# spotify/basic-pitch

Hardware: NVIDIA H100
Metric: audio_seconds_per_second (higher is better)
Workload: dtype f32

## Files before the change

basic_pitch_b200/csrc/kernels.cuh:

```cuda
#pragma once
#include <cuda_bf16.h>

#include <cstring>
#include <vector>

#include "common.cuh"

namespace bp {

void hcqt_setup();
constexpr int kLp2 = kTaps + 14;
struct Lowpass2 {
  float2 t[kLp2];
};
Lowpass2 lowpass_pairs(const float* h_lp );
void launch_decimate(const Lowpass2& lp, const float* audio, const WinDesc* desc, float* chain, int stage, int n_windows,
                     cudaStream_t st);
void launch_cqt(const float* audio, const WinDesc* desc, const float* chain, const float* wt, const float* scale,
                float* logmag, unsigned int* minmax, int n_windows, cudaStream_t st);
void launch_lognorm(float* y, const unsigned int* minmax, const float* bn , int n_windows,
                    cudaStream_t st);

struct CnnWeights {
  const float *contour1_wT, *contour1_b;
  const float *contour2_wT, *contour2_b;
  const float *note1_wT, *note1_b;
  const float *note2_wT, *note2_b;
  const float *onset1_wT, *onset1_b;
  const float *onset2_wT, *onset2_b;
};
void cnn_setup();
void launch_contour1(const float* y, const CnnWeights& w, float* c1, int n_windows, cudaStream_t st);
void launch_contour2(const float* c1, const CnnWeights& w, float* contour, int n_windows, cudaStream_t st);
void launch_note1(const float* contour, const CnnWeights& w, float* n1, int n_windows, cudaStream_t st);
void launch_note2(const float* n1, const CnnWeights& w, float* note, int n_windows, cudaStream_t st);
void launch_onset1(const float* y, const CnnWeights& w, float* o1, int n_windows, cudaStream_t st);
void launch_onset2(const float* note, const float* o1, const CnnWeights& w, float* onset, int n_windows,
                   cudaStream_t st);


struct TcConvSpec {
  int KH, KW, SF, PT, PL, COUT, FLT, WOUT;
  int n_ci;
  int shifts[8];
  int data_bins, chunks8;
  int rows_per_window, lead_rows;
  int layer;
  int KH2, HALO, G0;
  int n2_tiles, n2, js, width, pass;
  int W;
  int slot[24];
  __host__ __device__ constexpr int n_ft() const { return (WOUT + FLT - 1) / FLT; }
  __host__ __device__ constexpr int tile_bins() const { return 8 * (chunks8 - 1); }
  __host__ __device__ constexpr int ksteps() const { return (KH * n_ci * W + 15) / 16; }
  __host__ __device__ constexpr int edge_per_side() const { return 2 * HALO + (layer == 0 ? 8 - HALO : 0); }
};
__host__ __device__ constexpr TcConvSpec tc_spec(int layer) {
  return layer == 0 ? TcConvSpec{3, 39, 1, 1, 19, 8, 16, 264, 8, {-36, 0, 36, 57, 72, 84, 93, 101}, kCqtBins,     40, 174, 3, 0, 5, 2, 9,  1, 32, 5, 104, 40, 0, {}}
       : layer == 1 ? TcConvSpec{5, 5, 3, 2, 1, 32, 4, 88, 8, {-36, 0, 36, 57, 72, 84, 93, 101},   kCqtBins,     40, 174, 3, 1, 3, 1, 12, 2, 16, 4, 32, 32,   6,
                                 {9, 10, 21, 22, 14, 4, 2, 1, 16, 3, 6, 13, 5, 17, 18, 20, 19, 23, 7, 0, 8, 15, 12, 11}}
                    : TcConvSpec{7, 7, 3, 3, 2, 32, 4, 88, 1, {0, 0, 0, 0, 0, 0, 0, 0},           kContourBins, 34, 175, 6, 2, 7, 1, 12, 2, 32, 8, 64, 64,   8, {}};
}
struct TcConvPlan {
  TcConvSpec spec{};
  std::vector<uint16_t> tiles;
  std::vector<int> tile_seq;
  std::vector<uint32_t> slot_words[2];
  std::vector<int> group_step_off;
  std::vector<int> group_ft;
  int n_tiles = 0, n_groups = 0, n_uses = 0;
  void build(const TcConvSpec& spec, const float* w );
};
struct TcConvDev {
  int layer;
  const uint16_t* tiles;
  const uint16_t* b1;
  const uint16_t* b2;
  float bias1[32];
  float bias2;
  float note_w[9];
};
int tc_upload_program(const TcConvPlan& contour_plan, cudaStream_t st);
void tc_build_b1(int layer, const float* w, std::vector<uint16_t>& out, bool window8 = false);
struct TcGatherGeom {
  int K, n_ci, KH, wout;
  int K_packed;
  std::vector<int> starts, ranges;
  std::vector<int> kmap;
};
TcGatherGeom tc_gather_geometry(int layer);
void tc_build_b2(int layer, const float* w2, std::vector<uint16_t>& out);
void tc_build_b2_full(int layer, const float* w2, std::vector<uint16_t>& out);
int tc_rows_total(int n_windows, int rows_per_window);
size_t tc_edge_floats(const TcConvSpec& spec, int n_windows);
// ... 172 lines not shown
```

basic_pitch_b200/csrc/tc_conv.cu:

```cuda
#include <cuda.h>
#include <cuda_bf16.h>

#include <algorithm>
#include <cstdlib>
#include <cstring>
#include <unordered_map>
#include <vector>

#include "kernels.cuh"
#include "tc_ptx.cuh"

namespace bp {

namespace tc {
constexpr int kMTile = 64;
constexpr int kTileBytes = 8192;
constexpr int kMaxSteps = 1024;
constexpr int kMaxGroups = 15;
static_assert(tc_spec(0).G0 <= kMaxGroups, "contour groups in constant memory");
constexpr int kConsumerWarps = 8;
constexpr int kProducerWarp = 8;
constexpr int kThreads = 32 * kConsumerWarps + 128;
constexpr int kProducerRegs = 24;
constexpr int kConsumerRegs = 240;
static_assert(kProducerRegs + 2 * kConsumerRegs <= 3 * 168, "register pool of the CTA");
}

__host__ __device__ constexpr int tc_gather_k(TcConvSpec g, int dt, int ci, int j) {
  if (g.W == 8) return 8 * (dt * g.n_ci + ci) + j;
  int P = 0;
  while (g.slot[P] != 3 * ci + j / 2) ++P;
  return g.n_ci * g.W * dt + 2 * P + (j & 1);
}
__host__ __device__ constexpr bool tc_gather_slots_ok(TcConvSpec g) {
  if (g.W == 8) return true;
  if (g.W != 6 || g.n_ci != 8) return false;
  for (int p = 0; p < 24; ++p) {
    int n = 0;
    for (int P = 0; P < 24; ++P) n += g.slot[P] == p;
    if (n != 1) return false;
  }
  return true;
}
__host__ __device__ constexpr int tc_gather_slot_shift(TcConvSpec g, int P) { return g.shifts[g.slot[P] / 3]; }
__host__ __device__ constexpr int tc_gather_slot_pair(TcConvSpec g, int P) { return g.slot[P] % 3; }
static_assert(tc_gather_slots_ok(tc_spec(1)) && tc_gather_slots_ok(tc_spec(2)), "K slot map of the gather");
static_assert(tc_spec(1).ksteps() == 15 && tc_spec(2).ksteps() == 4, "K-steps per output bin");
__host__ __device__ constexpr int tc_gather_start(TcConvSpec g, int f, int ci) {
  return (g.SF * f - g.PL + g.shifts[ci]) & ~1;
}
__host__ __device__ constexpr int tc_gather_lo(TcConvSpec g, int ci) { return g.shifts[ci] > 0 ? g.shifts[ci] : 0; }
__host__ __device__ constexpr int tc_gather_hi(TcConvSpec g, int ci) {
// ... 26 lines not shown
  return s;
}
static_assert(tc_smem(0, false).stages == 12 && tc_smem(0, true).stages == 9, "weight-ring depth per layer");
static_assert(tc_smem(1, true).total() <= kMaxSmem && tc_smem(2, true).total() <= kMaxSmem, "onset / note shared memory");
constexpr uint32_t kUseFirstAcc = 1u << 15, kNoUse = 0xffffffffu;
}

static inline uint16_t f2bf(float x) {
  uint32_t u;
  memcpy(&u, &x, 4);
  if ((u & 0x7f800000u) == 0x7f800000u) return (uint16_t)(u >> 16);
  u += 0x7fffu + ((u >> 16) & 1u);
  return (uint16_t)(u >> 16);
}
static inline float bf2f(uint16_t h) {
  uint32_t u = (uint32_t)h << 16;
  float f;
  memcpy(&f, &u, 4);
  return f;
}

void TcConvPlan::build(const TcConvSpec& sp, const float* W ) {
  using namespace tc;
  spec = sp;
  tiles.clear();
  tile_seq.clear();
  slot_words[0].clear();
  slot_words[1].clear();
  group_step_off.clear();
  group_ft.clear();
  const int n_ft = sp.n_ft();
  const int data_rows = kMTile + sp.KH - 1;
  const int lbo16 = data_rows;
  const int stride = sp.G0;

  std::unordered_map<uint64_t, std::vector<int>> by_hash;
  int n_keys = 0;
  std::vector<uint16_t> scratch(kTileBytes / 2);
  std::vector<uint32_t> key(16 * 128), keys;
  auto find_or_add = [&](int dt, int c, int ft, int clip_lo) -> int {
    bool any = false;
    std::fill(scratch.begin(), scratch.end(), (uint16_t)0);
    std::fill(key.begin(), key.end(), 0u);
    for (int kk = clip_lo; kk < 16; ++kk) {
      const int u = 8 * c + kk;
      if (u >= sp.data_bins) continue;
      for (int n = 0; n < 128; ++n) {
        const int fl = n / sp.COUT, co = n % sp.COUT;
        const int f = ft * sp.FLT + fl;
        double acc = 0.0;
        uint32_t mask = 0;
        for (int ci = 0; ci < sp.n_ci; ++ci) {
          const int gg = u - sp.shifts[ci];
          const int df = gg - sp.SF * f + sp.PL;
          if (df < 0 || df >= sp.KW || gg < 0 || gg >= kContourBins) continue;
          acc += (double)W[((co * sp.n_ci + ci) * sp.KH + dt) * sp.KW + df];
          mask |= 1u << ci;
        }
        if (!mask) continue;
        key[kk * 128 + n] = 1u + (((uint32_t)(dt * 1024 + (u - sp.SF * f + 512)) << 8) | mask);
        const float w = (float)acc;
        const uint16_t hi = f2bf(w);
        const uint16_t lo = f2bf(w - bf2f(hi));
        const size_t o = (size_t)(kk >> 3) * 128 * 8 + (size_t)n * 8 + (kk & 7);
        scratch[o] = hi;
        scratch[2048 + o] = lo;
        any = true;
      }
    }
    if (!any) return -1;
    uint64_t h = 1469598103934665603ull;
    for (uint32_t v : key) h = (h ^ v) * 1099511628211ull;
    for (int id : by_hash[h])
      if (std::memcmp(keys.data() + (size_t)id * key.size(), key.data(), key.size() * 4) == 0) return id;
    tiles.insert(tiles.end(), scratch.begin(), scratch.end());
    keys.insert(keys.end(), key.begin(), key.end());
    by_hash[h].push_back(n_keys);
    return n_keys++;
  };

  group_step_off.push_back(0);
  n_uses = 0;
  for (int ft_a = 0; ft_a < stride; ++ft_a) {
    const int ft_b = ft_a + stride < n_ft ? ft_a + stride : -1;
    const int fts[2] = {ft_a, ft_b};
    group_ft.push_back(ft_a);
    group_ft.push_back(ft_b);
    struct Use {
      int tile, slot, c8, dt, off;
    };
    std::vector<Use> uses;
    for (int dt = 0; dt < sp.KH; ++dt) {
      std::vector<Use> cand;
      for (int slot = 0; slot < 2; ++slot) {
        const int ft = fts[slot];
        if (ft < 0) continue;
        std::vector<bool> need(sp.chunks8, false);
        for (int ci = 0; ci < sp.n_ci; ++ci)
          for (int fl = 0; fl < sp.FLT; ++fl) {
            const int f = ft * sp.FLT + fl;
            if (f >= sp.WOUT) continue;
            for (int df = 0; df < sp.KW; ++df) {
              const int gg = sp.SF * f - sp.PL + df, u = gg + sp.shifts[ci];
              if (gg < 0 || gg >= kContourBins || u < 0 || u >= sp.data_bins) continue;
              need[u / 8] = true;
            }
          }
        for (int c8 = 0; c8 < sp.chunks8;) {
          if (!need[c8]) {
            ++c8;
            continue;
          }
          const int c = std::min(c8, sp.chunks8 - 3);
          const int off = 8 * c - sp.SF * sp.FLT * ft;
          const int tile = find_or_add(dt, c, ft, 8 * (c8 - c));
          if (tile >= 0) cand.push_back(Use{tile, slot, c, dt, off});
          c8 += 2;
        }
      }
      std::stable_sort(cand.begin(), cand.end(), [](const Use& a, const Use& b) {
        return a.off != b.off ? a.off < b.off : (a.tile != b.tile ? a.tile < b.tile : a.slot < b.slot);
      });
      uses.insert(uses.end(), cand.begin(), cand.end());
    }
    struct Step {
      int tile;
      uint32_t w[2];
    };
    std::vector<Step> steps;
    size_t i = 0;
    while (i < uses.size()) {
      size_t j = i;
      while (j < uses.size() && uses[j].tile == uses[i].tile && (j == i || uses[j].slot != uses[j - 1].slot)) ++j;
      Step stp{uses[i].tile, {kNoUse, kNoUse}};
      for (size_t u = i; u < j; ++u) {
        stp.w[uses[u].slot] = (uint32_t)(uses[u].c8 * lbo16 + uses[u].dt);
        ++n_uses;
      }
      steps.push_back(stp);
      i = j;
    }
    std::stable_sort(steps.begin(), steps.end(), [](const Step& a, const Step& b) {
      auto cls = [](const Step& s) { return s.w[1] == kNoUse ? 0 : (s.w[0] == kNoUse ? 2 : 1); };
      return cls(a) < cls(b);
    });
    bool seen[2] = {false, false};
    for (Step& stp : steps) {
      for (int sl = 0; sl < 2; ++sl)
        if (stp.w[sl] != kNoUse) {
          if (!seen[sl]) stp.w[sl] |= kUseFirstAcc;
          seen[sl] = true;
        }
      tile_seq.push_back(stp.tile);
      slot_words[0].push_back(stp.w[0]);
      slot_words[1].push_back(stp.w[1]);
    }
    group_step_off.push_back((int)tile_seq.size());
  }
  n_tiles = n_keys;
  n_groups = (int)group_ft.size() / 2;
}

__constant__ uint32_t c_prog[2][tc::kMaxSteps];
__constant__ int c_tile_seq[tc::kMaxSteps];
__constant__ int c_group_step_off[tc::kMaxGroups + 1];
__constant__ int c_group_ft[2 * tc::kMaxGroups];

void tc_build_b2(int layer, const float* w2, std::vector<uint16_t>& out) {
  const TcConvSpec sp = tc_spec(layer);
  const int tile_elems = 2 * 16 * sp.n2, KW2 = 2 * sp.HALO + 1;
  out.assign((size_t)sp.n2_tiles * tile_elems, 0);
  for (int tl = 0; tl < sp.n2_tiles; ++tl)
    for (int kk = 0; kk < 16; ++kk)
      for (int n = 0; n < sp.n2; ++n) {
        const int jp = n / sp.js, dt = n - jp * sp.js;
        const int b = (16 * tl + kk) / sp.COUT, c = (16 * tl + kk) % sp.COUT, df = b + 2 * sp.HALO - jp;
        if (dt >= sp.KH2 || df < 0 || df >= KW2) continue;
        const float w = w2[((c + (layer == 1 ? 1 : 0)) * sp.KH2 + dt) * KW2 + df];
        const uint16_t hi = f2bf(w), lo = f2bf(w - bf2f(hi));
        const size_t o = (size_t)tl * tile_elems + (size_t)(kk >> 3) * sp.n2 * 8 + (size_t)n * 8 + (kk & 7);
        out[o] = hi;
        out[o + 16 * sp.n2] = lo;
      }
}

int tc_upload_program(const TcConvPlan& pl, cudaStream_t st) {
  if (pl.spec.layer != 0 || (int)pl.tile_seq.size() > tc::kMaxSteps - 1 || pl.n_groups != tc_spec(0).G0) return -1;
  for (int sl = 0; sl < 2; ++sl)
    cudaMemcpyToSymbolAsync(c_prog, pl.slot_words[sl].data(), pl.slot_words[sl].size() * 4, (size_t)sl * tc::kMaxSteps * 4,
                            cudaMemcpyHostToDevice, st);
  cudaMemcpyToSymbolAsync(c_tile_seq, pl.tile_seq.data(), pl.tile_seq.size() * 4, 0, cudaMemcpyHostToDevice, st);
  cudaMemcpyToSymbolAsync(c_group_step_off, pl.group_step_off.data(), pl.group_step_off.size() * 4, 0,
                          cudaMemcpyHostToDevice, st);
  cudaMemcpyToSymbolAsync(c_group_ft, pl.group_ft.data(), pl.group_ft.size() * 4, 0, cudaMemcpyHostToDevice, st);
  return cudaStreamSynchronize(st) == cudaSuccess ? 0 : -1;
}

void tc_build_b1(int layer, const float* W , std::vector<uint16_t>& out, bool window8) {
  const TcConvSpec g = tc_spec(layer);
  const int wn = window8 ? 8 : g.W;
  const size_t plane = (size_t)16 * ((g.KH * g.n_ci * wn + 15) / 16) * 32;
  out.assign(4 * plane, 0);
  for (int p = 0; p < 2; ++p)
    for (int dt = 0; dt < g.KH; ++dt)
      for (int ci = 0; ci < g.n_ci; ++ci) {
        const int o = g.SF * p - g.PL + g.shifts[ci] - tc_gather_start(g, p, ci);
        for (int j = 0; j < wn; ++j) {
          const int df = j - o, k = window8 ? 8 * (dt * g.n_ci + ci) + j : tc_gather_k(g, dt, ci, j);
          if (df < 0 || df >= g.KW) continue;
          for (int co = 0; co < 32; ++co) {
            const float w = W[((co * g.n_ci + ci) * g.KH + dt) * g.KW + df];
            const uint16_t hi = f2bf(w), lo = f2bf(w - bf2f(hi));
            const size_t e = ((size_t)(k >> 3) * 32 + co) * 8 + (k & 7);
            out[(2 * p) * plane + e] = hi;
            out[(2 * p + 1) * plane + e] = lo;
          }
        }
      }
}

TcGatherGeom tc_gather_geometry(int layer) {
  const TcConvSpec g = tc_spec(layer);
  TcGatherGeom r;
  r.K = 16 * ((g.KH * g.n_ci * 8 + 15) / 16);
  r.K_packed = 16 * g.ksteps();
  for (int k = 0; k < r.K_packed; ++k) {
    int hit[3] = {-1, -1, -1};
// ... 146 lines not shown
};
#endif

int tc_read_clocks(int layer, unsigned long long* out, bool reset) {
#ifdef BP_TC_CLOCKS
  if (layer < 0 || layer > 2) return -1;
  if (cudaMemcpyFromSymbol(out, g_tc_clocks, tc::kNumClk * sizeof(unsigned long long),
                           (size_t)layer * tc::kNumClk * sizeof(unsigned long long)) != cudaSuccess)
    return -1;
  if (reset) {
    static const unsigned long long zero[tc::kNumClk] = {};
    if (cudaMemcpyToSymbol(g_tc_clocks, zero, sizeof(zero), (size_t)layer * sizeof(zero)) != cudaSuccess) return -1;
  }
  return 0;
#else
  (void)layer, (void)out, (void)reset;
  return -1;
#endif
}

__device__ __forceinline__ void slot_barrier(int slot) {
  asm volatile("bar.sync %0, 128;" ::"r"(1 + slot) : "memory");
}


struct RowOut {
  float* raw;
  float* unw;
  __nv_bfloat16* chl;
  float* edge;
  const float* note_col;
  int t;
  bool ok;
  int e_lo, e_hi;
};

template <int LAYER>
__device__ __forceinline__ void finish_pitch_tile(const TcArgs& a, const RowOut& ro, float (&S)[6], float (&carry)[2], int ft,
                                                  bool first, bool last) {
  constexpr TcConvSpec L = tc_spec(LAYER);
  static_assert(L.FLT + 2 * L.HALO == 6 && L.HALO == 1, "sums and carry of a pitch tile");
  const bool lower = ft > 0;
  if (first) {
    if (lower && ro.edge) {
      float* e = ro.edge + (size_t)(ro.e_lo * 2 + 0) * L.edge_per_side() * a.edge_rows;
      e[0] = S[0];
      e[a.edge_rows] = S[1];
    }
  } else {
    S[0] += carry[0];
    S[1] += carry[1];
  }
  const int jlo = first ? (lower ? 2 * L.HALO : L.HALO) : 0;
  const int jhi = (ft == L.n_ft() - 1) ? L.FLT + L.HALO : L.FLT;
  if (ro.ok) {
    float nv[3][6];
    if constexpr (LAYER == 1) {
#pragma unroll
      for (int c = 0; c < 6; ++c) {
        const int f = L.FLT * ft - 2 + c;
        const bool fin = (unsigned)f < (unsigned)kPitches;
        const float* col = ro.note_col + (size_t)f * a.o.raw_rows;
#pragma unroll
        for (int r = 0; r < 3; ++r)
          nv[r][c] = (fin && (unsigned)(ro.t + r - 1) < (unsigned)kFrames) ? __ldg(col + r - 1) : 0.f;
      }
    }
#pragma unroll
    for (int j = 0; j < L.FLT + L.HALO; ++j) {
      if (j < jlo || j >= jhi) continue;
      const int f = L.FLT * ft - L.HALO + j;
      float x = S[j] + a.bias2;
      if constexpr (LAYER == 1) {
#pragma unroll
        for (int r = 0; r < 3; ++r)
#pragma unroll
          for (int df = 0; df < 3; ++df)
            if (j + df < 6) x = fmaf(nv[r][j + df], a.note_w[r * 3 + df], x);
      }
      const float v = sigmoidf_fast(x);
      if (ro.raw) ro.raw[(size_t)f * a.o.raw_rows] = v;
      if (ro.unw) ro.unw[(size_t)f * a.o.frame_stride] = v;
    }
  }
  carry[0] = S[L.FLT];
  carry[1] = S[L.FLT + 1];
  if (last && ft < L.n_ft() - 1 && ro.edge && ro.e_hi >= 0) {
    float* e = ro.edge + (size_t)(ro.e_hi * 2 + 1) * L.edge_per_side() * a.edge_rows;
    e[0] = S[L.FLT];
    e[a.edge_rows] = S[L.FLT + 1];
  }
}

__device__ __forceinline__ void store_contour_chunk(const TcArgs& a, const RowOut& ro, int chunk, const float (&v)[8]) {
  store_split8(v, ro.chl, (size_t)chunk * a.o.chl_rows * 8, (size_t)a.o.chl_chunks * a.o.chl_rows * 8);
  const float4 x0 = make_float4(v[0], v[1], v[2], v[3]), x1 = make_float4(v[4], v[5], v[6], v[7]);
  if (ro.raw) {
    float4* d = reinterpret_cast<float4*>(ro.raw + (size_t)chunk * a.o.raw_rows * 8);
    d[0] = x0;
    d[1] = x1;
  }
  if (ro.unw) {
    float4* d = reinterpret_cast<float4*>(ro.unw + (size_t)chunk * a.o.frame_stride * 8);
    d[0] = x0;
    d[1] = x1;
  }
}

__device__ __forceinline__ void finish_contour_tile(const TcArgs& a, const RowOut& ro, float (&S)[20], int ft, bool first,
                                                    bool last, float (&carry)[4], float (&hold)[6]) {
  constexpr TcConvSpec L = tc_spec(0);
  static_assert(L.FLT == 16 && L.HALO == 2 && L.edge_per_side() == 10, "sums, carry and edge values of a contour tile");
  const bool lower = ft > 0;
  if (first) {
    if (lower && ro.edge) {
      float* e = ro.edge + (size_t)(ro.e_lo * 2 + 0) * L.edge_per_side() * a.edge_rows;
#pragma unroll
      for (int k = 0; k < 4; ++k) e[(size_t)k * a.edge_rows] = S[k];
#pragma unroll
      for (int k = 0; k < 6; ++k) e[(size_t)(4 + k) * a.edge_rows] = sigmoidf_fast(S[4 + k] + a.bias2);
    }
  } else {
#pragma unroll
    for (int k = 0; k < 4; ++k) S[k] += carry[k];
  }
  float fin[16];
#pragma unroll
  for (int j = 0; j < 16; ++j) fin[j] = sigmoidf_fast(S[j] + a.bias2);
  if (ro.ok) {
    if (!first) {
      const float v[8] = {hold[0], hold[1], hold[2], hold[3], hold[4], hold[5], fin[0], fin[1]};
      store_contour_chunk(a, ro, 2 * ft - 1, v);
    }
    if (!first || !lower) {
      const float v[8] = {fin[2], fin[3], fin[4], fin[5], fin[6], fin[7], fin[8], fin[9]};
      store_contour_chunk(a, ro, 2 * ft, v);
    }
  }
#pragma unroll
  for (int k = 0; k < 6; ++k) hold[k] = fin[10 + k];
#pragma unroll
  for (int k = 0; k < 4; ++k) carry[k] = S[16 + k];
  if (last && ft < L.n_ft() - 1 && ro.edge && ro.e_hi >= 0) {
    float* e = ro.edge + (size_t)(ro.e_hi * 2 + 1) * L.edge_per_side() * a.edge_rows;
#pragma unroll
    for (int k = 0; k < 4; ++k) e[(size_t)k * a.edge_rows] = S[16 + k];
#pragma unroll
    for (int k = 0; k < 6; ++k) e[(size_t)(4 + k) * a.edge_rows] = fin[10 + k];
  }
}

template <int NW>
__device__ __forceinline__ void conv2_mma(float (&p)[NW / 2], const uint32_t (&ah)[32], const uint32_t (&al)[32], uint32_t b2) {
  constexpr uint32_t kPlane = 128u * NW * 2u;
#pragma unroll
  for (int ks = 0; ks < 8; ++ks) {
    const uint64_t bh = make_desc(b2 + (uint32_t)(2 * ks * NW * 16), NW * 16, 128);
    const uint64_t bl = make_desc(b2 + kPlane + (uint32_t)(2 * ks * NW * 16), NW * 16, 128);
    const uint32_t xh[4] = {ah[4 * ks], ah[4 * ks + 1], ah[4 * ks + 2], ah[4 * ks + 3]};
    const uint32_t xl[4] = {al[4 * ks], al[4 * ks + 1], al[4 * ks + 2], al[4 * ks + 3]};
    if constexpr (NW == 104) {
      wgmma_rs_n104(p, xh, bh, ks ? 1u : 0u);
      wgmma_rs_n104(p, xh, bl, 1u);
      wgmma_rs_n104(p, xl, bh, 1u);
    } else if constexpr (NW == 64) {
      wgmma_rs_n64(p, xh, bh, ks ? 1u : 0u);
      wgmma_rs_n64(p, xh, bl, 1u);
      wgmma_rs_n64(p, xl, bh, 1u);
    } else {
      wgmma_rs_n32(p, xh, bh, ks ? 1u : 0u);
      wgmma_rs_n32(p, xh, bl, 1u);
      wgmma_rs_n32(p, xl, bh, 1u);
    }
  }
}

template <int LAYER>
// ... 82 lines not shown
    gr.template load<(I + 2) % KS>(s_data, x[(I + 2) % 3]);
    clk.lap(kClkFull);
  }
  if constexpr (I + 1 < NST) gather_steps<LAYER, I + 1>(acc, gr, x, s_data, d0, ft, fr0, qd, clk);
}

template <int LAYER>
__device__ __forceinline__ void gather_conv1(float (&acc)[64], const unsigned char* s_data, uint32_t b1, int ft, int fr0, int qd,
                                             TcClocks& clk) {
  using namespace tc;
  static_assert(tc_spec(LAYER).ksteps() >= 2, "the first two K-steps are loaded up front, of the same bin");
  GatherRegs<LAYER> gr;
  const uint64_t d0 = make_desc(b1, 32 * 16, 128);
  uint32_t x[3][8];
  gr.setup(tc_spec(LAYER).FLT * ft, fr0, qd);
  gr.template load<0>(s_data, x[0]);
  gr.template load<1>(s_data, x[1]);
  clk.lap(kClkFull);
  gather_steps<LAYER, 0>(acc, gr, x, s_data, d0, ft, fr0, qd, clk);
  wgmma_wait<0>();
  reg_fence(acc);
  clk.lap(kClkMma);
}

template <int LAYER, bool FUSED>
__global__ void __launch_bounds__(tc::kThreads, 1) conv_tc_kernel(const __grid_constant__ TcArgs a) {
  using namespace tc;
  constexpr TcConvSpec L = tc_spec(LAYER);
  constexpr bool kFused = FUSED;
  constexpr bool kGather = LAYER != 0;
  static_assert(kFused || !kGather, "the onset and note epilogues always fuse the next conv");
  constexpr int NW = L.width, PC = L.pass, PS = PC + 1;
  static_assert(PC % 8 == 0 && PC % L.js == 0, "a staging pass holds whole fragment blocks and whole output offsets");
  constexpr int kDataRows = kMTile + L.KH - 1, kFt = L.n_ft();
  extern __shared__ __align__(128) unsigned char smem[];
  constexpr TcSmem SM = tc_smem(LAYER, FUSED);
  constexpr int kStages = SM.stages;
  static_assert(SM.total() <= kMaxSmem && kStages <= kMaxStages && (kGather || kStages >= 4), "dynamic shared memory per CTA");
  unsigned char* s_data = smem;
  unsigned char* s_w = smem + SM.data_bytes;
  unsigned char* s_b1 = s_w + kStages * kTileBytes;
  unsigned char* s_b2 = s_b1 + SM.b1_bytes;
  float* s_p = reinterpret_cast<float*>(s_b2 + SM.b2_bytes);
  uint64_t* bars = reinterpret_cast<uint64_t*>(reinterpret_cast<unsigned char*>(s_p) + SM.p_bytes);
  uint64_t* full_w = bars;
  uint64_t* empty_w = bars + kStages;
  uint64_t* data_full = bars + 2 * kStages;
  uint64_t* data_empty = data_full + 1;
  uint64_t* b2_full = data_empty + 1;
  uint64_t* b1_full = b2_full + 1;
  uint32_t* issued = reinterpret_cast<uint32_t*>(b1_full + 1);

  const int warp = __shfl_sync(0xffffffffu, (int)(threadIdx.x >> 5), 0);
  const int lane = threadIdx.x & 31;
  constexpr uint32_t lbo = kDataRows * 16u;
  constexpr uint32_t plane_bytes = (L.chunks8 - 1) * lbo;

  if (threadIdx.x == 0) {
    for (int s = 0; s < kStages; ++s) {
      mbar_init(full_w + s, 1);
      mbar_init(empty_w + s, kConsumerWarps);
    }
    mbar_init(data_full, 1);
    mbar_init(data_empty, kConsumerWarps);
    mbar_init(b2_full, 1);
    mbar_init(b1_full, 1);
    *issued = 0;
// ... 54 lines not shown
    }
    clk.lap(kClkProdOther);
    clk.flush(LAYER);
  } else {
    setmaxnreg_inc<kConsumerRegs>();
    const int slot = warp >> 2, wq = warp & 3, gq = lane >> 2, qd = lane & 3;
    const int tid = threadIdx.x & 127;
    const int fr0 = 16 * wq + gq;
    uint32_t stage = 0, ph_w = 0, ph_d = 0, n_fill = 0;
    const uint32_t a_hi = smem_u32(s_data), a_lo = a_hi + plane_bytes, w_base = smem_u32(s_w);
    const uint32_t* prog = c_prog[slot];
    float* sp_rows = s_p + slot * 64 * PS;
    if constexpr (kFused) mbar_wait_wd(b2_full, 0, 6);
    if constexpr (kGather) mbar_wait_wd(b1_full, 0, 7);
    for (int it = blockIdx.x; it < n_items; it += gridDim.x) {
      const int mt = it / a.n_split, spl = it % a.n_split;
      const int g0 = spl * L.G0 / a.n_split, g1 = (spl + 1) * L.G0 / a.n_split;
      bool live[2];
      int rb[2], rt[2];
#pragma unroll
      for (int rr = 0; rr < 2; ++rr) {
        const int m = mt * a.ms - a.h2 + fr0 + 8 * rr;
        rb[rr] = m >= 0 ? m / L.rows_per_window : 0;
        rt[rr] = m - rb[rr] * L.rows_per_window;
        live[rr] = m >= 0 && (rb[rr] < a.n_windows) && (rt[rr] < kFrames);
      }
      RowOut ro{};
      float carry[4] = {0.f, 0.f, 0.f, 0.f};
      float hold[6] = {0.f, 0.f, 0.f, 0.f, 0.f, 0.f};
      if constexpr (kFused) {
        const int row = tid;
        const int q = mt * a.ms - 2 * a.h2 + row;
        const int b = q >= 0 ? q / L.rows_per_window : 0, t = q - b * L.rows_per_window;
        ro.e_lo = slot * a.n_split + spl;
        ro.e_hi = (spl + 1 < a.n_split) ? slot * a.n_split + spl + 1 : (slot == 0 ? a.n_split : -1);
        ro.ok = row < 64 && row >= 2 * a.h2 && q >= 0 && b < a.n_windows && t < kFrames;
        ro.t = t;
        if (ro.ok) {
          ro.edge = a.o.edge + q;
          int uf = -1;
          if (a.o.ud) {
            const UnwrapDesc u = a.o.ud[b];
            const int tt = t - kOverlapHalf;
            if ((unsigned)tt < (unsigned)max(u.rows, 0)) uf = (int)(u.dst_base + tt);
          }
          if constexpr (LAYER == 0) {
            ro.chl = a.o.chl + ((size_t)a.o.chl_lead + (size_t)b * a.o.chl_rpw + t) * 8;
            if (a.o.raw) ro.raw = a.o.raw + ((size_t)b * kFrames + t) * 8;
            if (uf >= 0) ro.unw = a.o.unwrapped + (size_t)uf * 8;
          } else {
            if (a.o.raw) ro.raw = a.o.raw + (size_t)b * kFrames + t;
            if (uf >= 0) ro.unw = a.o.unwrapped + uf;
            if constexpr (LAYER == 1) ro.note_col = a.o.note_raw + (size_t)b * kFrames + t;
          }
        }
      }
      clk.lap(kClkConsOther);
      mbar_wait_wd(data_full, ph_d, 3);
      clk.lap(kClkData);
      ph_d ^= 1;
      for (int g = g0; g < g1; ++g) {
        float acc[64];
        int ft;
        if constexpr (kGather) {
          ft = g + slot * L.G0 < kFt ? g + slot * L.G0 : -1;
          if (ft >= 0) gather_conv1<LAYER>(acc, s_data, smem_u32(s_b1), ft, fr0, qd, clk);
        } else {
          ft = c_group_ft[2 * g + slot];
          const int s0 = c_group_step_off[g], s1 = c_group_step_off[g + 1];
          int pend = -1;
          uint32_t pend_fill = 0;
          uint32_t w = prog[s0];
          for (int s = s0; s < s1; ++s, ++n_fill) {
            const uint32_t w_next = prog[s + 1];
            if (w != kNoUse) {
              if (pend >= 0 && n_fill - pend_fill >= kStages) {
                wgmma_wait<0>();
                if (lane == 0) mbar_arrive(empty_w + pend);
                pend = -1;
              }
              clk.lap(kClkConsOther);
              counter_wait_above(issued, n_fill);
              mbar_wait_wd(full_w + stage, ph_w, 5);
              clk.lap(kClkFull);
              const uint32_t off = (w & 0x3fffu) << 4;
              const uint32_t bw = w_base + stage * kTileBytes;
              const uint64_t dah = make_desc(a_hi + off, lbo, 128), dal = make_desc(a_lo + off, lbo, 128);
              const uint64_t dbh = make_desc(bw, 2048, 128), dbl = make_desc(bw + 4096, 2048, 128);
              wgmma_fence();
              wgmma_ss_n128(acc, dah, dbh, (w & kUseFirstAcc) ? 0u : 1u);
              wgmma_ss_n128(acc, dah, dbl, 1u);
              wgmma_ss_n128(acc, dal, dbh, 1u);
              wgmma_commit();
              wgmma_wait<1>();
              if (pend >= 0 && lane == 0) mbar_arrive(empty_w + pend);
              pend = (int)stage;
              pend_fill = n_fill;
              clk.lap(kClkMma);
            }
            if (++stage == kStages) {
              stage = 0;
              ph_w ^= 1;
            }
            w = w_next;
          }
          clk.lap(kClkConsOther);
          wgmma_wait<0>();
          reg_fence(acc);
          clk.lap(kClkMma);
          if (pend >= 0 && lane == 0) mbar_arrive(empty_w + pend);
        }
        if (g == g1 - 1 && lane == 0) mbar_arrive(data_empty);
        if (ft < 0) continue;
        const bool first = (g == g0);
        const bool last = (g == g1 - 1) || (ft == kFt - 1);
        const int n_valid = min(L.FLT, L.WOUT - ft * L.FLT) * L.COUT;
        float bz[4][2];
#pragma unroll
        for (int i = 0; i < 4; ++i)
#pragma unroll
          for (int e = 0; e < 2; ++e) bz[i][e] = a.bias1[(8 * i + 2 * qd + e) % L.COUT];
        if constexpr (!kFused) {
#pragma unroll
          for (int rr = 0; rr < 2; ++rr) {
            if (!live[rr]) continue;
            float* dst = a.o.act + ((size_t)rb[rr] * kFrames + rt[rr]) * ((size_t)L.WOUT * L.COUT) + (size_t)ft * 128;
#pragma unroll
            for (int i = 0; i < 16; ++i) {
              const int col = 8 * i + 2 * qd;
              if (col < n_valid)
                *reinterpret_cast<float2*>(dst + col) = make_float2(fmaxf(acc[4 * i + 2 * rr] + bz[i & 3][0], 0.f),
                                                                    fmaxf(acc[4 * i + 2 * rr + 1] + bz[i & 3][1], 0.f));
            }
          }
        } else {
          uint32_t ah[32], al[32];
#pragma unroll
          for (int i = 0; i < 16; ++i)
#pragma unroll
            for (int rr = 0; rr < 2; ++rr) {
              const bool ok = live[rr] && 8 * i < n_valid;
              const float o0 = ok ? fmaxf(acc[4 * i + 2 * rr] + bz[i & 3][0], 0.f) : 0.f;
              const float o1 = ok ? fmaxf(acc[4 * i + 2 * rr + 1] + bz[i & 3][1], 0.f) : 0.f;
              const __nv_bfloat162 hh = __floats2bfloat162_rn(o0, o1);
              const uint32_t hu = *reinterpret_cast<const uint32_t*>(&hh);
              const __nv_bfloat162 ll =
                  __floats2bfloat162_rn(o0 - __uint_as_float(hu << 16), o1 - __uint_as_float(hu & 0xffff0000u));
              const int r = 4 * (i >> 1) + 2 * (i & 1) + rr;
// ... 27 lines not shown
#pragma unroll
              for (int j = q * JP; j < NJ && j < (q + 1) * JP; ++j) {
                float s = 0.f;
#pragma unroll
                for (int ta = 0; ta < KH2; ++ta)
                  if (tid - ta >= 0) s += sp_rows[(tid - ta) * PS + j * JS - q * PC + (KH2 - 1 - ta)];
                S[j] = s;
              }
            }
          }
          if (tid < 64) {
            if constexpr (LAYER == 0) {
              finish_contour_tile(a, ro, S, ft, first, last, carry, hold);
            } else {
              float c2[2] = {carry[0], carry[1]};
              finish_pitch_tile<LAYER>(a, ro, S, c2, ft, first, last);
              carry[0] = c2[0];
              carry[1] = c2[1];
            }
          }
        }
        clk.lap(kClkEpi);
      }
    }
    clk.lap(kClkConsOther);
    clk.flush(LAYER);
  }
}


struct EdgeFixArgs {
  TcOut o;
  int edge_rows, n_rows;
  int n_edges;
  int n_split, n_windows;
  float bias2, note_w[9];
};

template <int LAYER>
constexpr int kEdgeThreads = LAYER == 0 ? 1 : 2 * tc_spec(LAYER).HALO;

template <int LAYER>
__global__ void edge_fix_kernel(const EdgeFixArgs a) {
  constexpr TcConvSpec L = tc_spec(LAYER);
  const long long idx = (long long)blockIdx.x * blockDim.x + threadIdx.x;
  constexpr int per_edge = kEdgeThreads<LAYER>;
  const long long total = (long long)a.n_rows * a.n_edges * per_edge;
  if (idx >= total) return;
  const int R = (int)(idx % a.n_rows);
  const int ek = (int)(idx / a.n_rows);
  const int e = ek / per_edge, k = ek - e * per_edge;
  const int b = R / L.rows_per_window, t = R - b * L.rows_per_window;
  if (b >= a.n_windows || t >= kFrames) return;
  const int es = e / a.n_split, eq = e - es * a.n_split;
  const int ft_b = eq * L.G0 / a.n_split + es * L.G0;
  if (ft_b <= 0 || ft_b >= L.n_ft()) return;
  int uf = -1;
  if (a.o.ud) {
    const UnwrapDesc u = a.o.ud[b];
    const int tt = t - kOverlapHalf;
    if ((unsigned)tt < (unsigned)max(u.rows, 0)) uf = (int)(u.dst_base + tt);
  }
  if constexpr (LAYER == 0) {
    const float* lo = a.o.edge + (size_t)(e * 2 + 0) * L.edge_per_side() * a.edge_rows + R;
    const float* hi = a.o.edge + (size_t)(e * 2 + 1) * L.edge_per_side() * a.edge_rows + R;
    float fx[4];
#pragma unroll
    for (int q = 0; q < 4; ++q)
      fx[q] = sigmoidf_fast((lo[(size_t)q * a.edge_rows] + hi[(size_t)q * a.edge_rows]) + a.bias2);
    float va[8], vb[8];
#pragma unroll
    for (int q = 0; q < 6; ++q) {
      va[q] = hi[(size_t)(4 + q) * a.edge_rows];
      vb[2 + q] = lo[(size_t)(4 + q) * a.edge_rows];
    }
    va[6] = fx[0], va[7] = fx[1], vb[0] = fx[2], vb[1] = fx[3];
    __nv_bfloat16* chl = a.o.chl + ((size_t)a.o.chl_lead + (size_t)b * a.o.chl_rpw + t) * 8;
    const size_t plane = (size_t)a.o.chl_chunks * a.o.chl_rows * 8;
#pragma unroll
    for (int c = 0; c < 2; ++c) {
      const int chunk = 2 * ft_b - 1 + c;
      const float(&v)[8] = c ? vb : va;
      store_split8(v, chl, (size_t)chunk * a.o.chl_rows * 8, plane);
      const float4 x0 = make_float4(v[0], v[1], v[2], v[3]), x1 = make_float4(v[4], v[5], v[6], v[7]);
      if (a.o.raw) {
        float4* d = reinterpret_cast<float4*>(a.o.raw + ((size_t)chunk * a.o.raw_rows + (size_t)b * kFrames + t) * 8);
        d[0] = x0, d[1] = x1;
      }
      if (uf >= 0) {
        float4* d = reinterpret_cast<float4*>(a.o.unwrapped + ((size_t)chunk * a.o.frame_stride + uf) * 8);
        d[0] = x0, d[1] = x1;
      }
    }
    return;
  }
  const int f = L.FLT * ft_b - L.HALO + k;
  if (f < 0 || f >= L.WOUT) return;
  float x = (a.o.edge[((size_t)(e * 2 + 0) * L.edge_per_side() + k) * a.edge_rows + R] +
             a.o.edge[((size_t)(e * 2 + 1) * L.edge_per_side() + k) * a.edge_rows + R]) + a.bias2;
  if (a.o.note_raw) {
#pragma unroll
    for (int dt = 0; dt < 3; ++dt)
#pragma unroll
      for (int df = 0; df < 3; ++df) {
        const int tt = t + dt - 1, ff = f + df - 1;
        if ((unsigned)tt < (unsigned)kFrames && (unsigned)ff < (unsigned)kPitches)
          x = fmaf(__ldg(a.o.note_raw + (size_t)ff * a.o.raw_rows + (size_t)b * kFrames + tt), a.note_w[dt * 3 + df], x);
      }
  }
  const float v = sigmoidf_fast(x);
  if (a.o.raw) a.o.raw[(size_t)f * a.o.raw_rows + (size_t)b * kFrames + t] = v;
  if (uf >= 0) a.o.unwrapped[(size_t)f * a.o.frame_stride + uf] = v;
}
int tc_rows_total(int n_windows, int rows_per_window) {
  return n_windows * rows_per_window + tc::kMTile + 16;
}

int tc_setup() {
  using namespace tc;
  cudaError_t e = cudaFuncSetAttribute(conv_tc_kernel<0, false>, cudaFuncAttributeMaxDynamicSharedMemorySize, tc_smem(0, false).total());
  if (e == cudaSuccess) e = cudaFuncSetAttribute(conv_tc_kernel<1, true>, cudaFuncAttributeMaxDynamicSharedMemorySize, tc_smem(1, true).total());
  if (e == cudaSuccess) e = cudaFuncSetAttribute(conv_tc_kernel<2, true>, cudaFuncAttributeMaxDynamicSharedMemorySize, tc_smem(2, true).total());
  if (e == cudaSuccess) e = cudaFuncSetAttribute(conv_tc_kernel<0, true>, cudaFuncAttributeMaxDynamicSharedMemorySize, tc_smem(0, true).total());
  return e == cudaSuccess ? 0 : -1;
}

void launch_lognorm_split(const float* y, const unsigned int* minmax, const float* bn, __nv_bfloat16* dst,
                          const TcConvSpec& sp, int n_windows, int rows_stride, cudaStream_t st) {
  const int rows_used = tc_rows_total(n_windows, sp.rows_per_window);
  const long long cells = (long long)rows_used * (sp.chunks8 / 2);
  lognorm_split_kernel<<<(unsigned)((cells + 255) / 256), 256, 0, st>>>(y, minmax, bn, dst, n_windows, rows_used, rows_stride,
                                                                       sp.chunks8, sp.rows_per_window, sp.lead_rows);
}

size_t tc_edge_floats(const TcConvSpec& sp, int n_windows) {
  const int ms = tc::kMTile - (sp.KH2 - 1);
  const int n_mtiles = (n_windows * sp.rows_per_window + ms - 1) / ms;
  return (size_t)2 * sp.G0 * 2 * sp.edge_per_side() * ((size_t)n_mtiles * ms);
}

template <int LAYER, bool FUSED>
static void launch_layer(const TcArgs& a, const EdgeFixArgs& ef, int grid, cudaStream_t st) {
  conv_tc_kernel<LAYER, FUSED><<<grid, tc::kThreads, tc::tc_smem(LAYER, FUSED).total(), st>>>(a);
  if (FUSED) {
    const long long total = (long long)ef.n_rows * ef.n_edges * kEdgeThreads<LAYER>;
    edge_fix_kernel<LAYER><<<(unsigned)((total + 255) / 256), 256, 0, st>>>(ef);
  }
}

void launch_conv_tc(const __nv_bfloat16* data, const TcConvDev& dev, const TcOut& o, int n_windows, int rows_stride,
                    int n_sms, cudaStream_t st, bool fuse_next) {
  const TcConvSpec sp = tc_spec(dev.layer);
  const bool fused = dev.layer != 0 || fuse_next;
  TcArgs a{};
  a.data = data;
  a.tiles = dev.tiles;
  a.b1 = dev.b1;
  a.b2 = dev.b2;
  a.o = o;
  a.rows_total = rows_stride;
  a.h2 = fused ? (sp.KH2 - 1) / 2 : 0;
  a.ms = tc::kMTile - 2 * a.h2;
  a.n_mtiles = (n_windows * sp.rows_per_window + a.ms - 1) / a.ms;
  a.edge_rows = a.n_mtiles * a.ms;
  a.n_windows = n_windows;
  int split = 1;
  double best = 1e30;
  for (int s = 1; s <= sp.G0; ++s) {
    const int waves = (a.n_mtiles * s + n_sms - 1) / n_sms;
    const double cost = waves * ((sp.G0 + s - 1) / s + 0.5);
    if (cost < best - 1e-9) best = cost, split = s;
  }
  a.n_split = split;
  a.row0 = sp.lead_rows - sp.PT - a.h2;
  a.chunks8 = sp.chunks8;
  std::copy_n(dev.bias1, 32, a.bias1);
  a.bias2 = dev.bias2;
  std::copy_n(dev.note_w, 9, a.note_w);
  const int n_items = a.n_mtiles * a.n_split;
  const int grid = n_items < n_sms ? n_items : n_sms;
  {
    using EncodeFn = CUresult (*)(CUtensorMap*, CUtensorMapDataType, cuuint32_t, void*, const cuuint64_t*, const cuuint64_t*,
                                  const cuuint32_t*, const cuuint32_t*, CUtensorMapInterleave, CUtensorMapSwizzle,
                                  CUtensorMapL2promotion, CUtensorMapFloatOOBfill);
    static EncodeFn encode = [] {
      void* fn = nullptr;
      cudaDriverEntryPointQueryResult q;
      if (cudaGetDriverEntryPoint("cuTensorMapEncodeTiled", &fn, cudaEnableDefault, &q) != cudaSuccess ||
          q != cudaDriverEntryPointSuccess)
        fn = nullptr;
      return reinterpret_cast<EncodeFn>(fn);
    }();
    a.use_tmap = 0;
    static const bool want_tmap = getenv("BP_B200_TMAP") != nullptr;
    if (encode && want_tmap) {
      const cuuint64_t dims[4] = {8, (cuuint64_t)rows_stride, (cuuint64_t)sp.chunks8, 2};
      const cuuint64_t strides[3] = {16, (cuuint64_t)rows_stride * 16, (cuuint64_t)sp.chunks8 * rows_stride * 16};
      const cuuint32_t box[4] = {8, (cuuint32_t)(tc::kMTile + sp.KH - 1), (cuuint32_t)(sp.chunks8 - 1), 2};
      const cuuint32_t estr[4] = {1, 1, 1, 1};
      if (encode(&a.data_map, CU_TENSOR_MAP_DATA_TYPE_BFLOAT16, 4, const_cast<__nv_bfloat16*>(data), dims, strides, box, estr,
                 CU_TENSOR_MAP_INTERLEAVE_NONE, CU_TENSOR_MAP_SWIZZLE_NONE, CU_TENSOR_MAP_L2_PROMOTION_L2_128B,
                 CU_TENSOR_MAP_FLOAT_OOB_FILL_NONE) == CUDA_SUCCESS)
        a.use_tmap = 1;
    }
  }
  EdgeFixArgs ef{};
  ef.o = o;
  ef.edge_rows = a.edge_rows;
  ef.n_rows = n_windows * sp.rows_per_window;
  ef.n_edges = 2 * split;
  ef.n_split = split;
  ef.n_windows = n_windows;
  ef.bias2 = dev.bias2;
  std::copy_n(dev.note_w, 9, ef.note_w);
  if (dev.layer == 1)
    launch_layer<1, true>(a, ef, grid, st);
  else if (dev.layer == 2)
    launch_layer<2, true>(a, ef, grid, st);
  else if (fuse_next)
    launch_layer<0, true>(a, ef, grid, st);
  else
    launch_layer<0, false>(a, ef, grid, st);
}

}
```

Before: 140,400.

## Pair adjacent frequency tiles per group and fix only real range boundaries

Adds a PD parameter that defines a compile-time map from group and slot to frequency tile. The contour layer now pairs adjacent tiles rather than tiles a stride apart, and each pair's weight-step sequences are merged with an LCS so shared weight tiles are issued once for both slots. Edge writes and the edge-fix kernel are now keyed by tile boundary through a bitmask of boundaries that actually start a new range, so fewer boundaries are patched and each thread loops over the mask. The constant-memory group-to-tile table is removed. The risk is a changed summation order and a different step count per group, which can shift the tensor-core schedule.

```diff
diff --git a/basic_pitch_b200/csrc/kernels.cuh b/basic_pitch_b200/csrc/kernels.cuh
--- a/basic_pitch_b200/csrc/kernels.cuh
+++ b/basic_pitch_b200/csrc/kernels.cuh
@@ -47,6 +47,7 @@
   int rows_per_window, lead_rows;
   int layer;
   int KH2, HALO, G0;
+  int PD;
   int n2_tiles, n2, js, width, pass;
   int W;
   int slot[24];
@@ -56,10 +57,40 @@
   __host__ __device__ constexpr int edge_per_side() const { return 2 * HALO + (layer == 0 ? 8 - HALO : 0); }
 };
 __host__ __device__ constexpr TcConvSpec tc_spec(int layer) {
-  return layer == 0 ? TcConvSpec{3, 39, 1, 1, 19, 8, 16, 264, 8, {-36, 0, 36, 57, 72, 84, 93, 101}, kCqtBins,     40, 174, 3, 0, 5, 2, 9,  1, 32, 5, 104, 40, 0, {}}
-       : layer == 1 ? TcConvSpec{5, 5, 3, 2, 1, 32, 4, 88, 8, {-36, 0, 36, 57, 72, 84, 93, 101},   kCqtBins,     40, 174, 3, 1, 3, 1, 12, 2, 16, 4, 32, 32,   6,
+  return layer == 0 ? TcConvSpec{3, 39, 1, 1, 19, 8, 16, 264, 8, {-36, 0, 36, 57, 72, 84, 93, 101}, kCqtBins,     40, 174, 3, 0, 5, 2, 9,  1,  1, 32, 5, 104, 40, 0, {}}
+       : layer == 1 ? TcConvSpec{5, 5, 3, 2, 1, 32, 4, 88, 8, {-36, 0, 36, 57, 72, 84, 93, 101},   kCqtBins,     40, 174, 3, 1, 3, 1, 12, 12, 2, 16, 4, 32, 32,   6,
                                  {9, 10, 21, 22, 14, 4, 2, 1, 16, 3, 6, 13, 5, 17, 18, 20, 19, 23, 7, 0, 8, 15, 12, 11}}
-                    : TcConvSpec{7, 7, 3, 3, 2, 32, 4, 88, 1, {0, 0, 0, 0, 0, 0, 0, 0},           kContourBins, 34, 175, 6, 2, 7, 1, 12, 2, 32, 8, 64, 64,   8, {}};
+                    : TcConvSpec{7, 7, 3, 3, 2, 32, 4, 88, 1, {0, 0, 0, 0, 0, 0, 0, 0},           kContourBins, 34, 175, 6, 2, 7, 1, 12, 12, 2, 32, 8, 64, 64,   8, {}};
+}
+__host__ __device__ constexpr int tc_group_tile(const TcConvSpec& s, int g, int slot) {
+  if (g < 0 || g >= s.G0) return -1;
+  const int run = g / s.PD, i = g - run * s.PD, ft = 2 * s.PD * run + slot * s.PD + i;
+  return ft < s.n_ft() ? ft : -1;
+}
+__host__ __device__ constexpr int tc_tile_group(const TcConvSpec& s, int ft) {
+  const int run = ft / (2 * s.PD), r = ft - run * 2 * s.PD, slot = r / s.PD;
+  return ((run * s.PD + r - slot * s.PD) << 1) | slot;
+}
+__host__ __device__ constexpr bool tc_starts_range(const TcConvSpec& s, int g, int slot, bool item_start) {
+  const int ft = tc_group_tile(s, g, slot);
+  return item_start || ft <= 0 || tc_group_tile(s, g - 1, slot) != ft - 1;
+}
+__host__ __device__ constexpr bool tc_ends_range(const TcConvSpec& s, int g, int slot, bool item_end) {
+  return item_end || tc_group_tile(s, g + 1, slot) != tc_group_tile(s, g, slot) + 1;
+}
+__host__ __device__ constexpr bool tc_item_starts(const TcConvSpec& s, int n_split, int g) {
+  const int q = (g * n_split + s.G0 - 1) / s.G0;
+  return q < n_split && q * s.G0 / n_split == g;
+}
+__host__ __device__ constexpr bool tc_pairing_ok(const TcConvSpec& s) {
+  for (int ft = 0; ft < s.n_ft(); ++ft) {
+    int n = 0;
+    for (int g = 0; g < s.G0; ++g)
+      for (int slot = 0; slot < 2; ++slot) n += tc_group_tile(s, g, slot) == ft;
+    const int gs = tc_tile_group(s, ft);
+    if (n != 1 || tc_group_tile(s, gs >> 1, gs & 1) != ft) return false;
+  }
+  return true;
 }
 struct TcConvPlan {
   TcConvSpec spec{};
diff --git a/basic_pitch_b200/csrc/tc_conv.cu b/basic_pitch_b200/csrc/tc_conv.cu
--- a/basic_pitch_b200/csrc/tc_conv.cu
+++ b/basic_pitch_b200/csrc/tc_conv.cu
@@ -18,6 +18,10 @@
 constexpr int kMaxSteps = 1024;
 constexpr int kMaxGroups = 15;
 static_assert(tc_spec(0).G0 <= kMaxGroups, "contour groups in constant memory");
+static_assert(tc_pairing_ok(tc_spec(0)) && tc_pairing_ok(tc_spec(1)) && tc_pairing_ok(tc_spec(2)), "group -> tile map");
+static_assert(tc_spec(0).n_ft() <= 2 * tc_spec(0).G0 && tc_spec(1).n_ft() <= 2 * tc_spec(1).G0 &&
+                  tc_spec(2).n_ft() <= 2 * tc_spec(2).G0,
+              "every tile has a place in the reference pairing of the summation order (TcConvPlan::build)");
 constexpr int kConsumerWarps = 8;
 constexpr int kProducerWarp = 8;
 constexpr int kThreads = 32 * kConsumerWarps + 128;
@@ -110,7 +114,6 @@
   const int n_ft = sp.n_ft();
   const int data_rows = kMTile + sp.KH - 1;
   const int lbo16 = data_rows;
-  const int stride = sp.G0;
 
   std::unordered_map<uint64_t, std::vector<int>> by_hash;
   int n_keys = 0;
@@ -157,19 +160,23 @@
     return n_keys++;
   };
 
-  group_step_off.push_back(0);
-  n_uses = 0;
-  for (int ft_a = 0; ft_a < stride; ++ft_a) {
-    const int ft_b = ft_a + stride < n_ft ? ft_a + stride : -1;
-    const int fts[2] = {ft_a, ft_b};
-    group_ft.push_back(ft_a);
-    group_ft.push_back(ft_b);
-    struct Use {
+  struct Use {
+    int tile;
+    uint32_t w;
+  };
+  struct Step {
+    int tile;
+    uint32_t w[2];
+  };
+  std::vector<std::vector<Use>> order(n_ft);
+  for (int t = 0; t < sp.G0; ++t) {
+    const int fts[2] = {t, t + sp.G0 < n_ft ? t + sp.G0 : -1};
+    struct Cand {
       int tile, slot, c8, dt, off;
     };
-    std::vector<Use> uses;
+    std::vector<Cand> uses;
     for (int dt = 0; dt < sp.KH; ++dt) {
-      std::vector<Use> cand;
+      std::vector<Cand> cand;
       for (int slot = 0; slot < 2; ++slot) {
         const int ft = fts[slot];
         if (ft < 0) continue;
@@ -192,29 +199,22 @@
           const int c = std::min(c8, sp.chunks8 - 3);
           const int off = 8 * c - sp.SF * sp.FLT * ft;
           const int tile = find_or_add(dt, c, ft, 8 * (c8 - c));
-          if (tile >= 0) cand.push_back(Use{tile, slot, c, dt, off});
+          if (tile >= 0) cand.push_back(Cand{tile, slot, c, dt, off});
           c8 += 2;
         }
       }
-      std::stable_sort(cand.begin(), cand.end(), [](const Use& a, const Use& b) {
+      std::stable_sort(cand.begin(), cand.end(), [](const Cand& a, const Cand& b) {
         return a.off != b.off ? a.off < b.off : (a.tile != b.tile ? a.tile < b.tile : a.slot < b.slot);
       });
       uses.insert(uses.end(), cand.begin(), cand.end());
     }
-    struct Step {
-      int tile;
-      uint32_t w[2];
-    };
     std::vector<Step> steps;
     size_t i = 0;
     while (i < uses.size()) {
       size_t j = i;
       while (j < uses.size() && uses[j].tile == uses[i].tile && (j == i || uses[j].slot != uses[j - 1].slot)) ++j;
       Step stp{uses[i].tile, {kNoUse, kNoUse}};
-      for (size_t u = i; u < j; ++u) {
-        stp.w[uses[u].slot] = (uint32_t)(uses[u].c8 * lbo16 + uses[u].dt);
-        ++n_uses;
-      }
+      for (size_t u = i; u < j; ++u) stp.w[uses[u].slot] = (uint32_t)(uses[u].c8 * lbo16 + uses[u].dt);
       steps.push_back(stp);
       i = j;
     }
@@ -222,12 +222,44 @@
       auto cls = [](const Step& s) { return s.w[1] == kNoUse ? 0 : (s.w[0] == kNoUse ? 2 : 1); };
       return cls(a) < cls(b);
     });
+    for (const Step& stp : steps)
+      for (int sl = 0; sl < 2; ++sl)
+        if (stp.w[sl] != kNoUse) order[fts[sl]].push_back(Use{stp.tile, stp.w[sl]});
+  }
+
+  group_step_off.push_back(0);
+  n_uses = 0;
+  const std::vector<Use> none;
+  for (int g = 0; g < sp.G0; ++g) {
+    const int fts[2] = {tc_group_tile(sp, g, 0), tc_group_tile(sp, g, 1)};
+    group_ft.push_back(fts[0]);
+    group_ft.push_back(fts[1]);
+    const std::vector<Use>& a = fts[0] >= 0 ? order[fts[0]] : none;
+    const std::vector<Use>& b = fts[1] >= 0 ? order[fts[1]] : none;
+    const size_t na = a.size(), nb = b.size();
+    std::vector<int> lcs((na + 1) * (nb + 1), 0);
+    auto L = [&](size_t i, size_t j) -> int& { return lcs[i * (nb + 1) + j]; };
+    for (size_t i = na; i-- > 0;)
+      for (size_t j = nb; j-- > 0;)
+        L(i, j) = a[i].tile == b[j].tile ? 1 + L(i + 1, j + 1) : std::max(L(i + 1, j), L(i, j + 1));
     bool seen[2] = {false, false};
-    for (Step& stp : steps) {
+    for (size_t i = 0, j = 0; i < na || j < nb;) {
+      Step stp{-1, {kNoUse, kNoUse}};
+      if (i < na && j < nb && a[i].tile == b[j].tile) {
+        stp = Step{a[i].tile, {a[i].w, b[j].w}};
+        ++i, ++j;
+      } else if (j == nb || (i < na && L(i + 1, j) > L(i, j + 1))) {
+        stp = Step{a[i].tile, {a[i].w, kNoUse}};
+        ++i;
+      } else {
+        stp = Step{b[j].tile, {kNoUse, b[j].w}};
+        ++j;
+      }
       for (int sl = 0; sl < 2; ++sl)
         if (stp.w[sl] != kNoUse) {
           if (!seen[sl]) stp.w[sl] |= kUseFirstAcc;
           seen[sl] = true;
+          ++n_uses;
         }
       tile_seq.push_back(stp.tile);
       slot_words[0].push_back(stp.w[0]);
@@ -242,7 +274,6 @@
 __constant__ uint32_t c_prog[2][tc::kMaxSteps];
 __constant__ int c_tile_seq[tc::kMaxSteps];
 __constant__ int c_group_step_off[tc::kMaxGroups + 1];
-__constant__ int c_group_ft[2 * tc::kMaxGroups];
 
 void tc_build_b2(int layer, const float* w2, std::vector<uint16_t>& out) {
   const TcConvSpec sp = tc_spec(layer);
@@ -270,7 +301,6 @@
   cudaMemcpyToSymbolAsync(c_tile_seq, pl.tile_seq.data(), pl.tile_seq.size() * 4, 0, cudaMemcpyHostToDevice, st);
   cudaMemcpyToSymbolAsync(c_group_step_off, pl.group_step_off.data(), pl.group_step_off.size() * 4, 0,
                           cudaMemcpyHostToDevice, st);
-  cudaMemcpyToSymbolAsync(c_group_ft, pl.group_ft.data(), pl.group_ft.size() * 4, 0, cudaMemcpyHostToDevice, st);
   return cudaStreamSynchronize(st) == cudaSuccess ? 0 : -1;
 }
 
@@ -483,7 +513,6 @@
   const float* note_col;
   int t;
   bool ok;
-  int e_lo, e_hi;
 };
 
 template <int LAYER>
@@ -494,7 +523,7 @@
   const bool lower = ft > 0;
   if (first) {
     if (lower && ro.edge) {
-      float* e = ro.edge + (size_t)(ro.e_lo * 2 + 0) * L.edge_per_side() * a.edge_rows;
+      float* e = ro.edge + (size_t)((ft - 1) * 2 + 0) * L.edge_per_side() * a.edge_rows;
       e[0] = S[0];
       e[a.edge_rows] = S[1];
     }
@@ -536,8 +565,8 @@
   }
   carry[0] = S[L.FLT];
   carry[1] = S[L.FLT + 1];
-  if (last && ft < L.n_ft() - 1 && ro.edge && ro.e_hi >= 0) {
-    float* e = ro.edge + (size_t)(ro.e_hi * 2 + 1) * L.edge_per_side() * a.edge_rows;
+  if (last && ft < L.n_ft() - 1 && ro.edge) {
+    float* e = ro.edge + (size_t)(ft * 2 + 1) * L.edge_per_side() * a.edge_rows;
     e[0] = S[L.FLT];
     e[a.edge_rows] = S[L.FLT + 1];
   }
@@ -565,7 +594,7 @@
   const bool lower = ft > 0;
   if (first) {
     if (lower && ro.edge) {
-      float* e = ro.edge + (size_t)(ro.e_lo * 2 + 0) * L.edge_per_side() * a.edge_rows;
+      float* e = ro.edge + (size_t)((ft - 1) * 2 + 0) * L.edge_per_side() * a.edge_rows;
 #pragma unroll
       for (int k = 0; k < 4; ++k) e[(size_t)k * a.edge_rows] = S[k];
 #pragma unroll
@@ -592,8 +621,8 @@
   for (int k = 0; k < 6; ++k) hold[k] = fin[10 + k];
 #pragma unroll
   for (int k = 0; k < 4; ++k) carry[k] = S[16 + k];
-  if (last && ft < L.n_ft() - 1 && ro.edge && ro.e_hi >= 0) {
-    float* e = ro.edge + (size_t)(ro.e_hi * 2 + 1) * L.edge_per_side() * a.edge_rows;
+  if (last && ft < L.n_ft() - 1 && ro.edge) {
+    float* e = ro.edge + (size_t)(ft * 2 + 1) * L.edge_per_side() * a.edge_rows;
 #pragma unroll
     for (int k = 0; k < 4; ++k) e[(size_t)k * a.edge_rows] = S[16 + k];
 #pragma unroll
@@ -742,7 +771,7 @@
   static_assert(kFused || !kGather, "the onset and note epilogues always fuse the next conv");
   constexpr int NW = L.width, PC = L.pass, PS = PC + 1;
   static_assert(PC % 8 == 0 && PC % L.js == 0, "a staging pass holds whole fragment blocks and whole output offsets");
-  constexpr int kDataRows = kMTile + L.KH - 1, kFt = L.n_ft();
+  constexpr int kDataRows = kMTile + L.KH - 1;
   extern __shared__ __align__(128) unsigned char smem[];
   constexpr TcSmem SM = tc_smem(LAYER, FUSED);
   constexpr int kStages = SM.stages;
@@ -863,8 +892,6 @@
         const int row = tid;
         const int q = mt * a.ms - 2 * a.h2 + row;
         const int b = q >= 0 ? q / L.rows_per_window : 0, t = q - b * L.rows_per_window;
-        ro.e_lo = slot * a.n_split + spl;
-        ro.e_hi = (spl + 1 < a.n_split) ? slot * a.n_split + spl + 1 : (slot == 0 ? a.n_split : -1);
         ro.ok = row < 64 && row >= 2 * a.h2 && q >= 0 && b < a.n_windows && t < kFrames;
         ro.t = t;
         if (ro.ok) {
@@ -892,12 +919,10 @@
       ph_d ^= 1;
       for (int g = g0; g < g1; ++g) {
         float acc[64];
-        int ft;
+        const int ft = tc_group_tile(L, g, slot);
         if constexpr (kGather) {
-          ft = g + slot * L.G0 < kFt ? g + slot * L.G0 : -1;
           if (ft >= 0) gather_conv1<LAYER>(acc, s_data, smem_u32(s_b1), ft, fr0, qd, clk);
         } else {
-          ft = c_group_ft[2 * g + slot];
           const int s0 = c_group_step_off[g], s1 = c_group_step_off[g + 1];
           int pend = -1;
           uint32_t pend_fill = 0;
@@ -943,8 +968,8 @@
         }
         if (g == g1 - 1 && lane == 0) mbar_arrive(data_empty);
         if (ft < 0) continue;
-        const bool first = (g == g0);
-        const bool last = (g == g1 - 1) || (ft == kFt - 1);
+        const bool first = tc_starts_range(L, g, slot, g == g0);
+        const bool last = tc_ends_range(L, g, slot, g == g1 - 1);
         const int n_valid = min(L.FLT, L.WOUT - ft * L.FLT) * L.COUT;
         float bz[4][2];
 #pragma unroll
@@ -1038,35 +1063,30 @@
 struct EdgeFixArgs {
   TcOut o;
   int edge_rows, n_rows;
-  int n_edges;
-  int n_split, n_windows;
+  uint32_t edges;
+  int n_windows;
   float bias2, note_w[9];
 };
 
+__host__ __device__ constexpr uint32_t tc_edge_mask(const TcConvSpec& s, int n_split) {
+  uint32_t m = 0;
+  for (int b = 1; b < s.n_ft(); ++b) {
+    const int gs = tc_tile_group(s, b);
+    if (tc_starts_range(s, gs >> 1, gs & 1, tc_item_starts(s, n_split, gs >> 1))) m |= 1u << b;
+  }
+  return m;
+}
+static_assert(tc_spec(0).n_ft() <= 32 && tc_spec(1).n_ft() <= 32 && tc_spec(2).n_ft() <= 32, "boundary mask");
+static_assert(tc_edge_mask(tc_spec(0), 1) == 0x1fffeu && tc_edge_mask(tc_spec(1), 1) == 1u << 12,
+              "contour: every tile a range of its own; onset: the slot boundary only");
+
 template <int LAYER>
 constexpr int kEdgeThreads = LAYER == 0 ? 1 : 2 * tc_spec(LAYER).HALO;
 
 template <int LAYER>
-__global__ void edge_fix_kernel(const EdgeFixArgs a) {
+__device__ __forceinline__ void edge_fix_boundary(const EdgeFixArgs& a, int ft_b, int R, int b, int t, int uf, int k) {
   constexpr TcConvSpec L = tc_spec(LAYER);
-  const long long idx = (long long)blockIdx.x * blockDim.x + threadIdx.x;
-  constexpr int per_edge = kEdgeThreads<LAYER>;
-  const long long total = (long long)a.n_rows * a.n_edges * per_edge;
-  if (idx >= total) return;
-  const int R = (int)(idx % a.n_rows);
-  const int ek = (int)(idx / a.n_rows);
-  const int e = ek / per_edge, k = ek - e * per_edge;
-  const int b = R / L.rows_per_window, t = R - b * L.rows_per_window;
-  if (b >= a.n_windows || t >= kFrames) return;
-  const int es = e / a.n_split, eq = e - es * a.n_split;
-  const int ft_b = eq * L.G0 / a.n_split + es * L.G0;
-  if (ft_b <= 0 || ft_b >= L.n_ft()) return;
-  int uf = -1;
-  if (a.o.ud) {
-    const UnwrapDesc u = a.o.ud[b];
-    const int tt = t - kOverlapHalf;
-    if ((unsigned)tt < (unsigned)max(u.rows, 0)) uf = (int)(u.dst_base + tt);
-  }
+  const int e = ft_b - 1;
   if constexpr (LAYER == 0) {
     const float* lo = a.o.edge + (size_t)(e * 2 + 0) * L.edge_per_side() * a.edge_rows + R;
     const float* hi = a.o.edge + (size_t)(e * 2 + 1) * L.edge_per_side() * a.edge_rows + R;
@@ -1118,6 +1138,24 @@
   if (a.o.raw) a.o.raw[(size_t)f * a.o.raw_rows + (size_t)b * kFrames + t] = v;
   if (uf >= 0) a.o.unwrapped[(size_t)f * a.o.frame_stride + uf] = v;
 }
+
+template <int LAYER>
+__global__ void edge_fix_kernel(const EdgeFixArgs a) {
+  constexpr TcConvSpec L = tc_spec(LAYER);
+  const long long idx = (long long)blockIdx.x * blockDim.x + threadIdx.x;
+  if (idx >= (long long)a.n_rows * kEdgeThreads<LAYER>) return;
+  const int R = (int)(idx % a.n_rows);
+  const int k = (int)(idx / a.n_rows);
+  const int b = R / L.rows_per_window, t = R - b * L.rows_per_window;
+  if (b >= a.n_windows || t >= kFrames) return;
+  int uf = -1;
+  if (a.o.ud) {
+    const UnwrapDesc u = a.o.ud[b];
+    const int tt = t - kOverlapHalf;
+    if ((unsigned)tt < (unsigned)max(u.rows, 0)) uf = (int)(u.dst_base + tt);
+  }
+  for (uint32_t m = a.edges; m; m &= m - 1) edge_fix_boundary<LAYER>(a, __ffs(m) - 1, R, b, t, uf, k);
+}
 int tc_rows_total(int n_windows, int rows_per_window) {
   return n_windows * rows_per_window + tc::kMTile + 16;
 }
@@ -1142,14 +1180,14 @@
 size_t tc_edge_floats(const TcConvSpec& sp, int n_windows) {
   const int ms = tc::kMTile - (sp.KH2 - 1);
   const int n_mtiles = (n_windows * sp.rows_per_window + ms - 1) / ms;
-  return (size_t)2 * sp.G0 * 2 * sp.edge_per_side() * ((size_t)n_mtiles * ms);
+  return (size_t)(sp.n_ft() - 1) * 2 * sp.edge_per_side() * ((size_t)n_mtiles * ms);
 }
 
 template <int LAYER, bool FUSED>
 static void launch_layer(const TcArgs& a, const EdgeFixArgs& ef, int grid, cudaStream_t st) {
   conv_tc_kernel<LAYER, FUSED><<<grid, tc::kThreads, tc::tc_smem(LAYER, FUSED).total(), st>>>(a);
   if (FUSED) {
-    const long long total = (long long)ef.n_rows * ef.n_edges * kEdgeThreads<LAYER>;
+    const long long total = (long long)ef.n_rows * kEdgeThreads<LAYER>;
     edge_fix_kernel<LAYER><<<(unsigned)((total + 255) / 256), 256, 0, st>>>(ef);
   }
 }
@@ -1214,8 +1252,7 @@
   ef.o = o;
   ef.edge_rows = a.edge_rows;
   ef.n_rows = n_windows * sp.rows_per_window;
-  ef.n_edges = 2 * split;
-  ef.n_split = split;
+  ef.edges = tc_edge_mask(sp, split);
   ef.n_windows = n_windows;
   ef.bias2 = dev.bias2;
   std::copy_n(dev.note_w, 9, ef.note_w);
```

Result: faster. 147,100 (median of 6 runs) (+4.8%).
